# yjcaimeow/pointnerf

Hardware: AMD Instinct MI355X
Metric: Mray-samples/sec at 800x800, K=8, 2M neural points; PSNR delta vs ref (higher is better)
Workload: dtype fp32h2

## Files before the change

pointnerf_amd/csrc/aggregate_x3.hip:

```cpp
#include "agg_common.h"


namespace pnr {
namespace {

constexpr int kXT = 64;
constexpr int kXTS = kXT / kKN;
constexpr int kHidPlane = 32 * 64 * 16;
constexpr int kHidTile = 2 * kHidPlane;
constexpr int kXG = 34;
constexpr int kPG = 8;
constexpr int kPlaneX = kXG * kXT * 16;
constexpr int kPlaneP = kPG * kXT * 16;
constexpr int kP1Pitch = kHid + 4;

template <bool H>
struct XL {
  static constexpr int NPL = H ? 2 : 3;
  static constexpr int NPW = H ? 2 : 3;
  static constexpr unsigned kOne = H ? 0x3C00u : 0x3F80u;
  static constexpr int OffPE = NPL * kPlaneX;
  static constexpr int OffEx = OffPE + NPL * kPlaneP;
  static constexpr int NWB = H ? 3 : 2;
  static constexpr int OffWt = OffEx + 2 * 8 * kXT * 4;
  static constexpr int OffPr = OffWt + NWB * kXT * 4;
  static constexpr int OffSf = OffPr + 2 * kXT * 4;
  static constexpr int OffAp = OffSf + NWB * kXTS * 4;
  static constexpr int OffWa = OffAp + 4 * kXT * 4;
  static constexpr int OffH4 = OffWa + kHid * 4;
  static constexpr int OffTq = OffH4 + (H ? kXT * kP1Pitch * 4 : 0);
  static constexpr size_t Lds = (size_t)OffTq + 16;
  static_assert(OffSf % 16 == 0 && OffWa % 16 == 0 && OffH4 % 16 == 0, "16-B aligned LDS arrays");
  static_assert(kXT * kP1Pitch * 4 <= NPL * kPlaneX, "parked P1 fits the layer-input area");
  static_assert(Lds <= 160 * 1024, "LDS budget");
};

constexpr int kProducerPrio = 3;

typedef float f32x2n __attribute__((ext_vector_type(2)));
typedef float f32x4n __attribute__((ext_vector_type(4)));

struct X3Args {
  pnr_points pts;
  pnr_samples s;
  pnr_mlp w;
  SplitW wx;
  const float* p1;
  float* hid;
  int32_t* vmask;
  float* out_feat;
  float* out_weight;
  float* out_conf;
  int32_t* tile_ctr;
  pnr_agg_saved sv;
};

__device__ __forceinline__ bool xcd_mode(int64_t nt) { return nt >= 2 * (int64_t)gridDim.x + 16; }
__device__ __forceinline__ int64_t xcd_lo(int64_t nt, int x) { return nt * x / 8; }
__device__ __forceinline__ int64_t xcd_nb(int x) { return ((int)gridDim.x - x + 7) / 8; }

__device__ __forceinline__ int64_t first_tile(int64_t nt) {
  if (!xcd_mode(nt)) return blockIdx.x;
  return xcd_lo(nt, blockIdx.x & 7) + (blockIdx.x >> 3);
}

__device__ __forceinline__ int64_t take_tile(const X3Args& A, int64_t nt) {
  if (!xcd_mode(nt)) return (int64_t)gridDim.x + atomicAdd(A.tile_ctr, 1);
  const int x0 = blockIdx.x & 7;
  for (int i = 0; i < 8; ++i) {
    const int x = (x0 + i) & 7;
    const int64_t t = xcd_lo(nt, x) + xcd_nb(x) + atomicAdd(A.tile_ctr + x, 1);
    if (t < xcd_lo(nt, x + 1)) return t;
  }
  return nt;
}

__device__ __forceinline__ __amdgpu_buffer_rsrc_t rsrc(const void* base) {
  return __builtin_amdgcn_make_buffer_rsrc(const_cast<void*>(base), 0, 0x7fffffff, 0x00020000);
}

template <bool H, int NTK = 8>
__device__ __forceinline__ void load_w(uint4 (&a)[2][XL<H>::NPW], __amdgpu_buffer_rsrc_t rs, int voff, int t) {
  constexpr int NPW = XL<H>::NPW;
#pragma unroll
  for (int T = 0; T < 2; ++T)
#pragma unroll
    for (int pl = 0; pl < NPW; ++pl)
      a[T][pl] = __builtin_bit_cast(
          uint4, __builtin_amdgcn_raw_buffer_load_b128(
                     rs, voff + pl * 1024, (t * NTK + T) * NPW * 1024, 0));
}

template <bool H>
struct WRing {
  static constexpr int kWD = 3;
  uint4 a[kWD][2][XL<H>::NPW];
};

template <bool H, int NTK = 8>
__device__ __forceinline__ void prime(WRing<H>& w, __amdgpu_buffer_rsrc_t rs, int voff) {
#pragma unroll
  for (int d = 0; d < WRing<H>::kWD; ++d) load_w<H, NTK>(w.a[d], rs, voff, d);
}

template <bool H, int NTK = 8>
__device__ __forceinline__ void layer(f32x16 (&acc)[4], WRing<H>& w, __amdgpu_buffer_rsrc_t rs, int voff,
                                      const char* planes, int pstride, int nsteps, int lane) {
  constexpr int NPL = XL<H>::NPL, NPW = XL<H>::NPW, kWD = WRing<H>::kWD;
  const int c = lane & 31, h = lane >> 5;
  const char* base = planes + (h * kXT + c) * 16;
  auto ldb = [&](int t, int pt, uint4 (&bb)[NPL]) {
#pragma unroll
    for (int pl = 0; pl < NPL; ++pl)
      bb[pl] = *reinterpret_cast<const uint4*>(base + pl * pstride + (2 * t * kXT + 32 * pt) * 16);
  };
  constexpr int BD = H ? 2 : 1;
  uint4 b[BD][2][NPL];
#pragma unroll
  for (int sl = 0; sl < BD; ++sl) {
    const int t0 = sl < nsteps ? sl : nsteps - 1;
    ldb(t0, 0, b[sl][0]);
    ldb(t0, 1, b[sl][1]);
  }
  auto mm = [&](int pt, const uint4& av0, const uint4& av1, const uint4& bv) {
    if constexpr (H) {
      acc[2 * pt] = mfma_f16(av0, bv, acc[2 * pt]);
      acc[2 * pt + 1] = mfma_f16(av1, bv, acc[2 * pt + 1]);
    } else {
      acc[2 * pt] = mfma_bf16(av0, bv, acc[2 * pt]);
      acc[2 * pt + 1] = mfma_bf16(av1, bv, acc[2 * pt + 1]);
    }
  };
  auto wl = [&](uint4 (&a)[2][NPW], int pl, int tw) {
#pragma unroll
    for (int T = 0; T < 2; ++T)
      a[T][pl] = __builtin_bit_cast(
          uint4, __builtin_amdgcn_raw_buffer_load_b128(
                     rs, voff + pl * 1024, (tw * NTK + T) * NPW * 1024, 0));
  };
  auto bl = [&](int bs, int tn, int pt, int pl) {
    b[bs][pt][pl] = *reinterpret_cast<const uint4*>(base + pl * pstride + (2 * tn * kXT + 32 * pt) * 16);
  };
  uint4 scl[2];
  auto scale_next = [&](const uint4 (&an)[2][NPW], int T) {
    scl[T] = f16x8_scale2048(an[T][0]);
  };
  if constexpr (H) {
    scale_next(w.a[0], 0);
    scale_next(w.a[0], 1);
  }
  auto step_h = [&](uint4 (&a)[2][NPW], const uint4 (&an)[2][NPW], int t, int bs) {
    const int tn = t + BD < nsteps ? t + BD : nsteps - 1;
    const uint4 s0 = scl[0], s1 = scl[1];
#pragma unroll
    for (int pt = 0; pt < 2; ++pt) {
      mm(pt, s0, s1, b[bs][pt][0]);
      __builtin_amdgcn_sched_barrier(0);
      mm(pt, a[0][1], a[1][1], b[bs][pt][0]);
      __builtin_amdgcn_sched_barrier(0);
      if (pt == 1) wl(a, 1, t + kWD);
      if (pt == 0) scale_next(an, 0);
      bl(bs, tn, pt, 0);
      __builtin_amdgcn_sched_barrier(0);
      mm(pt, a[0][0], a[1][0], b[bs][pt][1]);
      __builtin_amdgcn_sched_barrier(0);
      bl(bs, tn, pt, 1);
      if (pt == 0) scale_next(an, 1);
      if (pt == 1) wl(a, 0, t + kWD);
      __builtin_amdgcn_sched_barrier(0);
    }
  };
  auto step = [&](uint4 (&a)[2][NPW], const uint4 (&an)[2][NPW], int t, int bs) {
    if constexpr (H) {
      step_h(a, an, t, bs);
    } else {
      const int tn = t + BD < nsteps ? t + BD : nsteps - 1;
#pragma unroll
      for (int pt = 0; pt < 2; ++pt) {
        mm(pt, a[0][2], a[1][2], b[bs][pt][0]);
        __builtin_amdgcn_sched_barrier(0);
        if (pt == 1) wl(a, 2, t + kWD);
        __builtin_amdgcn_sched_barrier(0);
        mm(pt, a[0][1], a[1][1], b[bs][pt][1]);
        mm(pt, a[0][0], a[1][0], b[bs][pt][2]);
        __builtin_amdgcn_sched_barrier(0);
        bl(bs, tn, pt, 2);
        __builtin_amdgcn_sched_barrier(0);
        mm(pt, a[0][1], a[1][1], b[bs][pt][0]);
        __builtin_amdgcn_sched_barrier(0);
        if (pt == 1) wl(a, 1, t + kWD);
        __builtin_amdgcn_sched_barrier(0);
        mm(pt, a[0][0], a[1][0], b[bs][pt][1]);
        __builtin_amdgcn_sched_barrier(0);
        bl(bs, tn, pt, 1);
        __builtin_amdgcn_sched_barrier(0);
        mm(pt, a[0][0], a[1][0], b[bs][pt][0]);
        __builtin_amdgcn_sched_barrier(0);
        bl(bs, tn, pt, 0);
        if (pt == 1) wl(a, 0, t + kWD);
        __builtin_amdgcn_sched_barrier(0);
      }
    }
  };
  constexpr int U = (BD == 2 && kWD % 2) ? 2 * kWD : kWD;
  int t = 0;
#pragma unroll 1
  for (; t + U <= nsteps; t += U) {
#pragma unroll
    for (int d = 0; d < U; ++d) step(w.a[d % kWD], w.a[(d + 1) % kWD], t + d, d % BD);
  }
#pragma unroll
  for (int d = 0; d < U - 1; ++d)
    if (t + d < nsteps) step(w.a[d % kWD], w.a[(d + 1) % kWD], t + d, d % BD);
}

__device__ __forceinline__ void lrelu_splith(float x0, float x1, float k, float ks, unsigned& hi, unsigned& lo) {
  typedef float f2 __attribute__((ext_vector_type(2)));
  const f2 x = {x0, x1};
  const f2 Y = __builtin_elementwise_max(x * k, x * ks);
  asm volatile(
      "v_fma_mixlo_f16 %0, %2, %4, 0\n\t"
      "v_fma_mixhi_f16 %0, %3, %4, 0\n\t"
      "v_fma_mixlo_f16 %1, %0, %5, %2 op_sel_hi:[1,0,0]\n\t"
      "v_fma_mixhi_f16 %1, %0, %5, %3 op_sel:[1,0,0] op_sel_hi:[1,0,0]"
      : "=&v"(hi), "=&v"(lo)
      : "v"(Y.x), "v"(Y.y), "s"(0x1p-11f), "s"(-2048.f));
}

template <bool H>
__device__ __forceinline__ void store_act(const f32x16 (&acc)[4], char* planes, float s, float mul, int lane,
                                          int T0, int pstride = kPlaneX) {
  const int c = lane & 31, h = lane >> 5;
  if constexpr (H) {
    const float k = 2048.f * mul, ks = k * s;
#pragma unroll
    for (int pt = 0; pt < 2; ++pt)
#pragma unroll
      for (int T = 0; T < 2; ++T)
#pragma unroll
        for (int q = 0; q < 4; ++q) {
          const f32x16& v = acc[2 * pt + T];
          unsigned a0, a1, b0, b1;
          lrelu_splith(v[4 * q], v[4 * q + 1], k, ks, a0, a1);
          lrelu_splith(v[4 * q + 2], v[4 * q + 3], k, ks, b0, b1);
          char* d = planes + ((4 * (T0 + T) + q) * kXT + 32 * pt + c) * 16 + 8 * h;
          *reinterpret_cast<uint2*>(d) = make_uint2(a0, b0);
          *reinterpret_cast<uint2*>(d + pstride) = make_uint2(a1, b1);
        }
    return;
  }
#pragma unroll
  for (int pt = 0; pt < 2; ++pt)
#pragma unroll
    for (int T = 0; T < 2; ++T)
#pragma unroll
      for (int q = 0; q < 4; ++q) {
        const f32x16& v = acc[2 * pt + T];
        unsigned a0, a1, a2, b0, b1, b2;
        split2(fmaxf(v[4 * q], s * v[4 * q]), fmaxf(v[4 * q + 1], s * v[4 * q + 1]), a0, a1, a2);
        split2(fmaxf(v[4 * q + 2], s * v[4 * q + 2]), fmaxf(v[4 * q + 3], s * v[4 * q + 3]), b0, b1, b2);
        char* d = planes + ((4 * (T0 + T) + q) * kXT + 32 * pt + c) * 16 + 8 * h;
        *reinterpret_cast<uint2*>(d) = make_uint2(a0, b0);
        *reinterpret_cast<uint2*>(d + kPlaneX) = make_uint2(a1, b1);
        *reinterpret_cast<uint2*>(d + 2 * kPlaneX) = make_uint2(a2, b2);
      }
}

template <bool H>
__device__ __forceinline__ void acc_init(f32x16 (&acc)[4], const float* bias, float inv_scale, int lane, int T0) {
  if constexpr (H) {
    const int h = lane >> 5;
#pragma unroll
    for (int T = 0; T < 2; ++T)
#pragma unroll
      for (int q = 0; q < 4; ++q) {
        const float4 b = *reinterpret_cast<const float4*>(bias + 32 * (T0 + T) + 8 * q + 4 * h);
        const float v[4] = {b.x * inv_scale, b.y * inv_scale, b.z * inv_scale, b.w * inv_scale};
#pragma unroll
        for (int i = 0; i < 4; ++i) {
          acc[T][4 * q + i] = v[i];
          acc[2 + T][4 * q + i] = v[i];
        }
      }
  } else {
#pragma unroll
    for (int i = 0; i < 4; ++i) acc[i] = (f32x16){0.f};
  }
}
constexpr int kBiasSteps(bool H) { return H ? 16 : 17; }

template <bool H>
__device__ __forceinline__ void store_group(char* planes, int pstride, int g, int pair, const float (&v)[8]) {
  if constexpr (H) {
    uint4 p0, p1;
    splith(v[0], v[1], p0.x, p1.x);
    splith(v[2], v[3], p0.y, p1.y);
    splith(v[4], v[5], p0.z, p1.z);
    splith(v[6], v[7], p0.w, p1.w);
    char* d = planes + (g * kXT + pair) * 16;
    *reinterpret_cast<uint4*>(d) = p0;
    *reinterpret_cast<uint4*>(d + pstride) = p1;
    return;
  }
  uint4 p0, p1, p2;
  split2(v[0], v[1], p0.x, p1.x, p2.x);
  split2(v[2], v[3], p0.y, p1.y, p2.y);
  split2(v[4], v[5], p0.z, p1.z, p2.z);
  split2(v[6], v[7], p0.w, p1.w, p2.w);
  char* d = planes + (g * kXT + pair) * 16;
  *reinterpret_cast<uint4*>(d) = p0;
  *reinterpret_cast<uint4*>(d + pstride) = p1;
  *reinterpret_cast<uint4*>(d + 2 * pstride) = p2;
}

struct GatherState {
  int64_t tile;
  int64_t row;
  int pid;
  float sw[3], sp[3];
  int64_t dmap;
  bool active;
};

__device__ __forceinline__ void gather_row(const X3Args& A, int64_t tile, int lane, GatherState& g) {
  const int64_t v = tile * kXTS + (lane >> 3);
  g.tile = tile;
  g.active = v < eff_n(A.s);
  g.row = g.active ? sample_row(A.s, v) : 0;
}

__device__ __forceinline__ void gather_sample(const X3Args& A, int lane, GatherState& g) {
  const int k = lane & 7, K = A.s.K;
  g.pid = (g.active && k < K) ? A.s.pidx[g.row * K + k] : -1;
#pragma unroll
  for (int a = 0; a < 3; ++a) {
    g.sw[a] = g.active ? A.s.sample_w[g.row * 3 + a] : 0.f;
    g.sp[a] = g.active ? A.s.sample_p[g.row * 3 + a] : 0.f;
  }
  g.dmap = A.s.dir_map ? (int64_t)A.s.dir_map[g.row] : g.row;
}

template <bool H, bool TR = false>
__device__ __forceinline__ void gather(const X3Args& A, const GatherState& g, int nb, int nw, char* lds, int pw, int lane,
                                       float (&dr6)[6]) {
  using L = XL<H>;
  float Rw[9];
#pragma unroll
  for (int i = 0; i < 9; ++i) Rw[i] = A.w.rw2c ? A.w.rw2c[i] : (i % 4 == 0 ? 1.f : 0.f);
// ... 130 lines not shown
    float s0, c0, s1, c1, s2, c2, s3, c3, s4, c4;
    sincosf(dr6[ch], &s0, &c0);
    sincosf(dr6[ch] * 2.f, &s1, &c1);
    sincosf(dr6[ch] * 4.f, &s2, &c2);
    sincosf(dr6[ch] * 8.f, &s3, &c3);
    sincosf(dr6[ch] * 16.f, &s4, &c4);
    pe_store<H>(lds, lane, 5 * ch + 0, s0, c0);
    pe_store<H>(lds, lane, 5 * ch + 1, s1, c1);
    pe_store<H>(lds, lane, 5 * ch + 2, s2, c2);
    pe_store<H>(lds, lane, 5 * ch + 3, s3, c3);
    pe_store<H>(lds, lane, 5 * ch + 4, s4, c4);
    if (TR && pe5) {
      const float sv[10] = {s0, c0, s1, c1, s2, c2, s3, c3, s4, c4};
#pragma unroll
      for (int i = 0; i < 10; i += 2) *reinterpret_cast<float2*>(pe5 + 10 * ch + i) = make_float2(sv[i], sv[i + 1]);
    }
  }
}

#define X3_SYNC() __syncthreads()

template <bool H, bool TR = false>
__device__ __forceinline__ void finalize_alpha(const X3Args& A, char* lds, int buf, int64_t tile, int lane) {
  using L = XL<H>;
  const int64_t n = eff_n(A.s);
  const int j = lane >> 3, k = lane & 7;
  const float* apart = reinterpret_cast<const float*>(lds + L::OffAp);
  const float* wtL = reinterpret_cast<const float*>(lds + L::OffWt) + buf * kXT;
  const int* sflag = reinterpret_cast<const int*>(lds + L::OffSf) + buf * kXTS;
  const float pa = apart[lane] + apart[kXT + lane] + apart[2 * kXT + lane] + apart[3 * kXT + lane] + A.w.ba[0];
  const float alpha_k = A.w.act_super ? softplus(pa - 1.f) : fmaxf(pa, 0.f);
  const float alpha_s = xor8_sum(wtL[lane] * alpha_k);
  const int64_t vo = tile * kXTS + j;
  if (TR && vo < n) A.sv.pa[tile * kXT + lane] = pa;
  if (k == 0 && vo < n) {
    A.vmask[vo] = sflag[j];
    if (sflag[j]) A.out_feat[vo * (kC + 1)] = alpha_s;
  }
}

template <bool H>
__device__ __forceinline__ void save_act_train(const X3Args& A, const f32x16 (&acc)[4], float* dst, int layer,
                                               int64_t tile, int64_t n, float neg, int lane, int T0, float sc) {
  const int c = lane & 31, h = lane >> 5;
#pragma unroll
  for (int pt = 0; pt < 2; ++pt) {
    const int col = 32 * pt + c;
    if (tile * kXTS + (col >> 3) >= n) continue;
    const int64_t pr = tile * kXT + col;
#pragma unroll
    for (int T = 0; T < 2; ++T) {
      f32x16 v = acc[2 * pt + T];
      if constexpr (H) v = v * sc;
      unsigned bits = 0;
#pragma unroll
      for (int q = 0; q < 4; ++q)
        *reinterpret_cast<float4*>(dst + pr * kHid + 32 * (T0 + T) + 8 * q + 4 * h) =
            make_float4(lrelu(v[4 * q], neg), lrelu(v[4 * q + 1], neg), lrelu(v[4 * q + 2], neg),
                        lrelu(v[4 * q + 3], neg));
#pragma unroll
      for (int r = 0; r < 16; ++r) bits |= (v[r] > 0.f ? 1u : 0u) << r;
      A.sv.mask[pr * 64 + 16 * layer + 2 * (T0 + T) + h] = (uint16_t)bits;
    }
  }
}

template <bool H, bool TR = false>
__device__ __forceinline__ void consumer_loop(const X3Args& A, char* lds, int wid, int lane) {
  using L = XL<H>;
  const int c = lane & 31, h = lane >> 5;
  const int64_t n = eff_n(A.s);
  const int64_t ntiles = cdiv(n, kXTS);
  const float neg = A.w.neg_slope;
  char* XP = lds;
  const char* PE = lds + L::OffPE;
  const float* P1L = reinterpret_cast<const float*>(lds);
  float* apart = reinterpret_cast<float*>(lds + L::OffAp);
  const float* waL = reinterpret_cast<const float*>(lds + L::OffWa);
  const int T0 = 2 * wid;
  const int voff = (T0 * L::NPW * 64 + lane) * 16;
  const __amdgpu_buffer_rsrc_t r1 = rsrc(A.wx.pack[0]), r2 = rsrc(A.wx.pack[1]), r3 = rsrc(A.wx.pack[2]),
                               r4 = rsrc(A.wx.pack[3]);
  const float sc1 = A.wx.scale[0], sc2 = A.wx.scale[1], sc3 = A.wx.scale[2], sc4 = A.wx.scale[3];
  WRing<H> wr;
  f32x16 acc[4];
  prime<H>(wr, r1, voff);
  X3_SYNC();
  const int* TQ = reinterpret_cast<const int*>(lds + L::OffTq);
  int it = 0;
  for (int64_t tile = first_tile(ntiles); tile < ntiles; tile = TQ[(it + 1) & 3], ++it) {
    const int buf = it & 1;
#pragma unroll
    for (int i = 0; i < 4; ++i) acc[i] = (f32x16){0.f};
    layer<H>(acc, wr, r1, voff, PE, kPlaneP, 4, lane);
    prime<H>(wr, r2, voff);
    X3_SYNC();
#pragma unroll
    for (int pt = 0; pt < 2; ++pt)
#pragma unroll
      for (int T = 0; T < 2; ++T)
#pragma unroll
        for (int q = 0; q < 4; ++q) {
          const float4 v4 = *reinterpret_cast<const float4*>(P1L + (32 * pt + c) * kP1Pitch + 32 * (T0 + T) + 8 * q +
                                                             4 * h);
          if constexpr (H) {
            acc[2 * pt + T][4 * q] = fmaf(acc[2 * pt + T][4 * q], sc1, v4.x);
            acc[2 * pt + T][4 * q + 1] = fmaf(acc[2 * pt + T][4 * q + 1], sc1, v4.y);
            acc[2 * pt + T][4 * q + 2] = fmaf(acc[2 * pt + T][4 * q + 2], sc1, v4.z);
            acc[2 * pt + T][4 * q + 3] = fmaf(acc[2 * pt + T][4 * q + 3], sc1, v4.w);
          } else {
            acc[2 * pt + T][4 * q] += v4.x;
            acc[2 * pt + T][4 * q + 1] += v4.y;
            acc[2 * pt + T][4 * q + 2] += v4.z;
            acc[2 * pt + T][4 * q + 3] += v4.w;
          }
        }
    X3_SYNC();
    store_act<H>(acc, XP, neg, 1.f, lane, T0);
    if constexpr (TR) save_act_train<H>(A, acc, A.sv.h1, 0, tile, n, neg, lane, T0, 1.f);
    if (wid == 0) {
#pragma unroll
      for (int pl = 0; pl < L::NPL; ++pl) {
        *reinterpret_cast<uint4*>(XP + pl * kPlaneX + (32 * kXT + lane) * 16) =
            make_uint4(pl == 0 ? L::kOne : 0u, 0u, 0u, 0u);
        *reinterpret_cast<uint4*>(XP + pl * kPlaneX + (33 * kXT + lane) * 16) = make_uint4(0u, 0u, 0u, 0u);
      }
    }
    acc_init<H>(acc, A.w.b2, 1.f / sc2, lane, T0);
    X3_SYNC();
    layer<H>(acc, wr, r2, voff, XP, kPlaneX, kBiasSteps(H), lane);
    prime<H>(wr, r3, voff);
    X3_SYNC();
    store_act<H>(acc, XP, neg, sc2, lane, T0);
    if constexpr (TR) save_act_train<H>(A, acc, A.sv.h2, 1, tile, n, neg, lane, T0, sc2);
    if (wid == 0) {
      const float* exL = reinterpret_cast<const float*>(lds + L::OffEx) + buf * 8 * kXT;
      float ex[8];
#pragma unroll
      for (int e = 0; e < 8; ++e) ex[e] = exL[e * kXT + lane];
      store_group<H>(XP, kPlaneX, 32, lane, ex);
    }
#pragma unroll
    for (int i = 0; i < 4; ++i) acc[i] = (f32x16){0.f};
    X3_SYNC();
    layer<H>(acc, wr, r3, voff, XP, kPlaneX, 17, lane);
    prime<H>(wr, r4, voff);
    X3_SYNC();
    store_act<H>(acc, XP, neg, sc3, lane, T0);
    if constexpr (TR) save_act_train<H>(A, acc, A.sv.h3, 2, tile, n, neg, lane, T0, sc3);
    if (wid == 0 && !H) {
#pragma unroll
      for (int pl = 0; pl < L::NPL; ++pl)
        *reinterpret_cast<uint4*>(XP + pl * kPlaneX + (32 * kXT + lane) * 16) =
            make_uint4(pl == 0 ? L::kOne : 0u, 0u, 0u, 0u);
    }
    acc_init<H>(acc, A.w.b4, 1.f / sc4, lane, T0);
    X3_SYNC();
    layer<H>(acc, wr, r4, voff, XP, kPlaneX, kBiasSteps(H), lane);
    prime<H>(wr, r1, voff);
    if constexpr (H) {
      if constexpr (TR) save_act_train<H>(A, acc, A.sv.h4, 3, tile, n, neg, lane, T0, sc4);
      float* H4 = reinterpret_cast<float*>(lds + L::OffH4);
#pragma unroll
      for (int pt = 0; pt < 2; ++pt)
#pragma unroll
        for (int T = 0; T < 2; ++T)
#pragma unroll
          for (int q = 0; q < 4; ++q) {
            const f32x16& v = acc[2 * pt + T];
            *reinterpret_cast<float4*>(H4 + (32 * pt + c) * kP1Pitch + 32 * (T0 + T) + 8 * q + 4 * h) =
                make_float4(v[4 * q], v[4 * q + 1], v[4 * q + 2], v[4 * q + 3]);
          }
    } else {
      if constexpr (TR) save_act_train<H>(A, acc, A.sv.h4, 3, tile, n, neg, lane, T0, 1.f);
      const float* wtL = reinterpret_cast<const float*>(lds + L::OffWt) + buf * kXT;
      const int* sflag = reinterpret_cast<const int*>(lds + L::OffSf) + buf * kXTS;
      float pa_part[2] = {0.f, 0.f};
      const int i8 = c & 7;
      const bool b2 = (i8 & 4) != 0, b1 = (i8 & 2) != 0, b0 = (i8 & 1) != 0;
#pragma unroll
      for (int pt = 0; pt < 2; ++pt) {
        const float wtp = wtL[32 * pt + c];
        const int sj = (32 * pt + c) >> 3;
        const int64_t vo = tile * kXTS + sj;
        const bool wrt = vo < n && sflag[sj];
#pragma unroll
        for (int T = 0; T < 2; ++T) {
          float v[16];
#pragma unroll
          for (int r = 0; r < 16; ++r) {
            const float hv = lrelu(H ? acc[2 * pt + T][r] * sc4 : acc[2 * pt + T][r], neg);
            pa_part[pt] += waL[32 * (T0 + T) + acc_row(r, h)] * hv;
            v[r] = wtp * hv;
          }
          float w8[8], w4[4], w2[2];
#pragma unroll
          for (int q = 0; q < 8; ++q) {
            const float send = b2 ? v[q] : v[q + 8];
            const float recv = __builtin_bit_cast(
                float, __builtin_amdgcn_mov_dpp(__builtin_bit_cast(int, send), 0x141, 0xf, 0xf, false));
            w8[q] = (b2 ? v[q + 8] : v[q]) + recv;
          }
#pragma unroll
          for (int q = 0; q < 4; ++q) {
            const float send = b1 ? w8[q] : w8[q + 4];
            const float recv = __builtin_bit_cast(
                float, __builtin_amdgcn_mov_dpp(__builtin_bit_cast(int, send), 0x4E, 0xf, 0xf, false));
            w4[q] = (b1 ? w8[q + 4] : w8[q]) + recv;
          }
#pragma unroll
          for (int q = 0; q < 2; ++q) {
            const float send = b0 ? w4[q] : w4[q + 2];
            const float recv = __builtin_bit_cast(
                float, __builtin_amdgcn_mov_dpp(__builtin_bit_cast(int, send), 0xB1, 0xf, 0xf, false));
            w2[q] = (b0 ? w4[q + 2] : w4[q]) + recv;
          }
          if (wrt)
            __builtin_nontemporal_store(
                (f32x2n){w2[0], w2[1]},
                reinterpret_cast<f32x2n*>(A.hid + vo * kHid + 32 * (T0 + T) + ((2 * i8) & 3) + 8 * (i8 >> 1) + 4 * h));
        }
        pa_part[pt] += __shfl_xor(pa_part[pt], 32);
      }
      if (h == 0) {
        apart[wid * kXT + c] = pa_part[0];
        apart[wid * kXT + 32 + c] = pa_part[1];
      }
    }
    X3_SYNC();
  }
}

__device__ __forceinline__ unsigned fetch_p1(f32x4n (&r)[16], const X3Args& A, const int* prow, int pw, int lane) {
  int64_t rows[16];
#pragma unroll
  for (int i = 0; i < 16; ++i) {
    const int pr = prow[16 * pw + i];
    rows[i] = pr < 0 ? -1 : (A.pts.used_map ? (int64_t)A.pts.used_map[pr] : (int64_t)pr);
  }
  unsigned empty = 0;
#pragma unroll
  for (int i = 0; i < 16; ++i) {
    r[i] = __builtin_nontemporal_load(reinterpret_cast<const f32x4n*>(A.p1 + (rows[i] < 0 ? 0 : rows[i]) * kHid) +
                                      lane);
    if (rows[i] < 0) empty |= 1u << i;
  }
  return empty;
}

__device__ __forceinline__ void park_p1(const f32x4n (&r)[16], unsigned empty, char* lds, int pw, int lane) {
  float* P1L = reinterpret_cast<float*>(lds);
#pragma unroll
  for (int i = 0; i < 16; ++i) {
    const f32x4n z = {0.f, 0.f, 0.f, 0.f};
// ... 287 lines not shown
      pe[24] = 1.f;
#pragma unroll
      for (int i = 25; i < 32; ++i) pe[i] = 0.f;
#pragma unroll
      for (int q = 0; q < 4; ++q) {
        const float g8[8] = {pe[8 * q], pe[8 * q + 1], pe[8 * q + 2], pe[8 * q + 3],
                             pe[8 * q + 4], pe[8 * q + 5], pe[8 * q + 6], pe[8 * q + 7]};
        store_group<true>(lds, kCPlane, 14 + q, lane, g8);
      }
    }
    __syncthreads();
    layer<true, 4>(acc, wr, r1b, voff, lds, kCPlane, 9, lane);
    prime<true, 4>(wr, r2, voff);
    __syncthreads();
    if (TR) save_act_rows(acc, A.hc[0], v0, n, neg, A.scale[0], lane, T0);
    store_act<true>(acc, lds, neg, A.scale[0], lane, T0, kCPlane);
    acc_init<true>(acc, A.w.bc2, 1.f / A.scale[1], lane, T0);
    __syncthreads();
    layer<true, 4>(acc, wr, r2, voff, lds, kCPlane, 8, lane);
    prime<true, 4>(wr, r3, voff);
    __syncthreads();
    if (TR) save_act_rows(acc, A.hc[1], v0, n, neg, A.scale[1], lane, T0);
    store_act<true>(acc, lds, neg, A.scale[1], lane, T0, kCPlane);
    acc_init<true>(acc, A.w.bc3, 1.f / A.scale[2], lane, T0);
    __syncthreads();
    layer<true, 4>(acc, wr, r3, voff, lds, kCPlane, 8, lane);
    prime<true, 4>(wr, r1a, voff);
    const float sc3 = A.scale[2];
    if (TR) save_act_rows(acc, A.hc[2], v0, n, neg, sc3, lane, T0);
#pragma unroll
    for (int i = 0; i < 4; ++i)
      if ((vm >> (32 * (i >> 1) + c)) & 1)
#pragma unroll
        for (int r = 0; r < 16; r += 2) chk = fmaf(0.f, acc[i][r] + acc[i][r + 1], chk);
    __syncthreads();
    float* Ob = reinterpret_cast<float*>(lds);
#pragma unroll
    for (int pt = 0; pt < 2; ++pt)
#pragma unroll
      for (int T = 0; T < 2; ++T)
#pragma unroll
        for (int q = 0; q < 4; ++q) {
          const f32x16& a = acc[2 * pt + T];
          *reinterpret_cast<float4*>(Ob + (32 * pt + c) * kOPitch + 32 * (T0 + T) + 8 * q + 4 * h) =
              make_float4(lrelu(a[4 * q] * sc3, neg), lrelu(a[4 * q + 1] * sc3, neg), lrelu(a[4 * q + 2] * sc3, neg),
                          lrelu(a[4 * q + 3] * sc3, neg));
        }
    __syncthreads();
    for (int r = wid; r < kXT; r += 2) {
      if (!((vm >> r) & 1)) continue;
      float* o = A.out_feat + (v0 + r) * (kC + 1) + 1;
      o[lane] = Ob[r * kOPitch + lane];
      o[64 + lane] = Ob[r * kOPitch + 64 + lane];
    }
    __syncthreads();
  }
  if (A.range_flag && chk != 0.f) atomicOr(A.range_flag, 1);
}

constexpr int kPG1 = 30;
constexpr int kP1Plane = kPG1 * kXT * 16;
constexpr size_t kP1H2Lds = 2 * (size_t)kP1Plane;

struct P1H2Args {
  pnr_points pts;
  const void* pack;
  float scale;
  int32_t* range_flag;
  float* p1;
  float* x1;
};

__global__ void __launch_bounds__(256) __attribute__((amdgpu_waves_per_eu(2, 2))) k_point_pre_h2(P1H2Args A) {
  extern __shared__ __attribute__((aligned(16))) char lds[];
  const int lane = threadIdx.x & 63, wid = threadIdx.x >> 6;
  const int c = lane & 31, h = lane >> 5;
  const int64_t np = p1_rows(A.pts);
  const int64_t ntiles = cdiv(np, kXT);
  const int T0 = 2 * wid;
  const int voff = (T0 * XL<true>::NPW * 64 + lane) * 16;
  const __amdgpu_buffer_rsrc_t rw = rsrc(A.pack);
  float chk = 0.f;
  WRing<true> wr;
  f32x16 acc[4];
  prime<true>(wr, rw, voff);
  for (int64_t tile = blockIdx.x; tile < ntiles; tile += gridDim.x) {
    {
      const int64_t pt = tile * kXT + lane;
      const bool act = pt < np;
      const int64_t prow = act ? (A.pts.used ? (int64_t)A.pts.used[pt] : pt) : 0;
      float e[8] = {0.f, 0.f, 0.f, 0.f, 0.f, 0.f, 0.f, 0.f};
      if (act) {
        const float4 a = reinterpret_cast<const float4*>(A.pts.emb + prow * kEmb + 8 * wid)[0];
        const float4 b = reinterpret_cast<const float4*>(A.pts.emb + prow * kEmb + 8 * wid)[1];
        e[0] = a.x; e[1] = a.y; e[2] = a.z; e[3] = a.w; e[4] = b.x; e[5] = b.y; e[6] = b.z; e[7] = b.w;
      }
      store_group<true>(lds, kP1Plane, wid, lane, e);
      if (A.x1 && act) {
        float4* xr = reinterpret_cast<float4*>(A.x1 + pt * 224 + 8 * wid);
        xr[0] = make_float4(e[0], e[1], e[2], e[3]);
        xr[1] = make_float4(e[4], e[5], e[6], e[7]);
      }
      float pe[48];
#pragma unroll
      for (int u = 0; u < 8; ++u) {
        float s0, c0;
        sincosf(e[u], &s0, &c0);
        const float s1 = 2.f * s0 * c0, c1 = (c0 - s0) * (c0 + s0);
        const float s2 = 2.f * s1 * c1, c2 = (c1 - s1) * (c1 + s1);
        pe[6 * u] = s0; pe[6 * u + 1] = c0; pe[6 * u + 2] = s1;
        pe[6 * u + 3] = c1; pe[6 * u + 4] = s2; pe[6 * u + 5] = c2;
      }
#pragma unroll
      for (int g = 0; g < 6; ++g) {
        const float g8[8] = {pe[8 * g], pe[8 * g + 1], pe[8 * g + 2], pe[8 * g + 3],
                             pe[8 * g + 4], pe[8 * g + 5], pe[8 * g + 6], pe[8 * g + 7]};
        store_group<true>(lds, kP1Plane, 4 + 6 * wid + g, lane, g8);
      }
      if (A.x1 && act) {
        float4* xr = reinterpret_cast<float4*>(A.x1 + pt * 224 + 32 + 48 * wid);
#pragma unroll
        for (int q = 0; q < 12; ++q) xr[q] = make_float4(pe[4 * q], pe[4 * q + 1], pe[4 * q + 2], pe[4 * q + 3]);
      }
      if (wid == 0) {
        const float one[8] = {1.f, 0.f, 0.f, 0.f, 0.f, 0.f, 0.f, 0.f};
        const float zero[8] = {0.f, 0.f, 0.f, 0.f, 0.f, 0.f, 0.f, 0.f};
        store_group<true>(lds, kP1Plane, 28, lane, one);
        store_group<true>(lds, kP1Plane, 29, lane, zero);
      }
    }
    __syncthreads();
#pragma unroll
    for (int i = 0; i < 4; ++i) acc[i] = (f32x16){0.f};
    layer<true>(acc, wr, rw, voff, lds, kP1Plane, 15, lane);
    prime<true>(wr, rw, voff);
#pragma unroll
    for (int pt = 0; pt < 2; ++pt) {
      const int64_t prow = tile * kXT + 32 * pt + c;
#pragma unroll
      for (int T = 0; T < 2; ++T)
#pragma unroll
        for (int q = 0; q < 4; ++q) {
          const f32x16& v = acc[2 * pt + T];
          const float4 o = make_float4(v[4 * q] * A.scale, v[4 * q + 1] * A.scale, v[4 * q + 2] * A.scale,
                                       v[4 * q + 3] * A.scale);
          chk = fmaf(0.f, (o.x + o.y) + (o.z + o.w), chk);
          if (prow < np)
            *reinterpret_cast<float4*>(A.p1 + prow * kHid + 32 * (T0 + T) + 8 * q + 4 * h) = o;
        }
    }
    __syncthreads();
  }
  if (A.range_flag && chk != 0.f) atomicOr(A.range_flag, 1);
}

}

int launch_point_pre_h2(const pnr_points& pts, const void* pack, float scale, int32_t* range_flag, float* p1,
                        hipStream_t st, float* x1) {
  static bool attr = false;
  if (!attr) {
    PNR_HIP(hipFuncSetAttribute(reinterpret_cast<const void*>(&k_point_pre_h2),
                                hipFuncAttributeMaxDynamicSharedMemorySize, (int)kP1H2Lds));
    attr = true;
  }
  P1H2Args a;
  a.pts = pts;
  a.pack = pack;
  a.scale = scale;
  a.range_flag = range_flag;
  a.p1 = p1;
  a.x1 = x1;
  const int64_t np = pts.used ? pts.n_used : pts.n;
  hipLaunchKernelGGL(k_point_pre_h2, dim3(grid_for(cdiv(np, kXT), 1, 256 * 2)), dim3(256), kP1H2Lds, st, a);
  PNR_LAUNCH_CHECK();
  return PNR_OK;
}

int launch_color_h2(const pnr_samples& s, const pnr_mlp& w, const void* const pack[4], const float scale[3],
                    int32_t* range_flag, const float* hid, const int32_t* vmask, float* out_feat, hipStream_t st,
                    const float* rw2c_pp, const pnr_agg_saved* train) {
  static bool attr = false;
  if (!attr) {
    PNR_HIP(hipFuncSetAttribute(reinterpret_cast<const void*>(&k_color_h2<false>),
                                hipFuncAttributeMaxDynamicSharedMemorySize, (int)kColH2Lds));
    PNR_HIP(hipFuncSetAttribute(reinterpret_cast<const void*>(&k_color_h2<true>),
                                hipFuncAttributeMaxDynamicSharedMemorySize, (int)kColH2Lds));
    attr = true;
  }
  ColH2Args a;
  a.s = s;
  a.w = w;
  for (int i = 0; i < 4; ++i) a.pack[i] = pack[i];
  for (int i = 0; i < 3; ++i) a.scale[i] = scale[i];
  a.range_flag = range_flag;
  a.hid = hid;
  a.vmask = vmask;
  a.out_feat = out_feat;
  a.rw2c_pp = rw2c_pp;
  a.hid_rows = train ? train->hid : nullptr;
  a.vpe = train ? train->vpe : nullptr;
  a.hc[0] = train ? train->hc1 : nullptr;
  a.hc[1] = train ? train->hc2 : nullptr;
  a.hc[2] = train ? train->hc3 : nullptr;
  const dim3 grid(grid_for(cdiv(s.n_max, kXT), 1, 256 * 4));
  if (train) hipLaunchKernelGGL(k_color_h2<true>, grid, dim3(128), kColH2Lds, st, a);
  else hipLaunchKernelGGL(k_color_h2<false>, grid, dim3(128), kColH2Lds, st, a);
  PNR_LAUNCH_CHECK();
  return PNR_OK;
}


template <bool H>
int launch_pairs_split(const pnr_points& pts, const pnr_samples& s, const pnr_mlp& w, const SplitW& wx,
                       const float* p1, float* hid, int32_t* vmask, float* out_feat, float* out_weight,
                       float* out_conf, int32_t* tile_ctr, hipStream_t st, const pnr_agg_saved* sv) {
  const void* fn = H ? (sv ? reinterpret_cast<const void*>(&k_pairs_h2_train) : reinterpret_cast<const void*>(&k_pairs_h2))
                     : (sv ? reinterpret_cast<const void*>(&k_pairs_x3_train) : reinterpret_cast<const void*>(&k_pairs_x3));
  static bool attr[2] = {false, false};
  if (!attr[sv ? 1 : 0]) {
    PNR_HIP(hipFuncSetAttribute(fn, hipFuncAttributeMaxDynamicSharedMemorySize, (int)XL<H>::Lds));
    attr[sv ? 1 : 0] = true;
  }
  X3Args a;
  a.pts = pts;
  a.s = s;
  a.w = w;
  a.wx = wx;
// ... 31 lines not shown
```

Baseline: 819.1.

## Use separate main and correction accumulators for f16 split MFMA layers

For the f16 two-plane weight split, the hi-plane product goes into its own accumulator set and the lo-plane products into a second correction set. The two sets are folded with a single fma (main*2048 + corr) at store time. This replaces the per-step rescaling of weights by 2048 (the scale_next VALU work) and starts from zero accumulators instead of explicit zeroing. The cost is 64 more accumulator VGPRs per lane, which risks spills or lower occupancy under the fixed waves-per-EU bound, and it changes how rounding errors accumulate.

```diff
diff --git a/pointnerf_amd/csrc/aggregate_x3.hip b/pointnerf_amd/csrc/aggregate_x3.hip
--- a/pointnerf_amd/csrc/aggregate_x3.hip
+++ b/pointnerf_amd/csrc/aggregate_x3.hip
@@ -103,9 +103,11 @@
   for (int d = 0; d < WRing<H>::kWD; ++d) load_w<H, NTK>(w.a[d], rs, voff, d);
 }
 
-template <bool H, int NTK = 8>
-__device__ __forceinline__ void layer(f32x16 (&acc)[4], WRing<H>& w, __amdgpu_buffer_rsrc_t rs, int voff,
-                                      const char* planes, int pstride, int nsteps, int lane) {
+template <bool H, int NTK = 8, bool ACC2 = false, bool ZACC = false>
+__device__ __forceinline__ void layer(f32x16 (&acc)[4], f32x16 (&corr)[4], WRing<H>& w, __amdgpu_buffer_rsrc_t rs,
+                                      int voff, const char* planes, int pstride, int nsteps, int lane) {
+  static_assert(ACC2 || !ZACC, "zero-start accumulators: with two accumulator sets only");
+  static_assert(H || !ACC2, "two accumulator sets: the f16 split only");
   constexpr int NPL = XL<H>::NPL, NPW = XL<H>::NPW, kWD = WRing<H>::kWD;
   const int c = lane & 31, h = lane >> 5;
   const char* base = planes + (h * kXT + c) * 16;
@@ -122,8 +124,13 @@
     ldb(t0, 0, b[sl][0]);
     ldb(t0, 1, b[sl][1]);
   }
-  auto mm = [&](int pt, const uint4& av0, const uint4& av1, const uint4& bv) {
-    if constexpr (H) {
+  auto mm = [&](int pt, const uint4& av0, const uint4& av1, const uint4& bv, bool to_corr = false, bool zc = false) {
+    if constexpr (ACC2) {
+      f32x16 (&d)[4] = to_corr ? corr : acc;
+      const f32x16 z = {0.f};
+      d[2 * pt] = mfma_f16(av0, bv, zc ? z : d[2 * pt]);
+      d[2 * pt + 1] = mfma_f16(av1, bv, zc ? z : d[2 * pt + 1]);
+    } else if constexpr (H) {
       acc[2 * pt] = mfma_f16(av0, bv, acc[2 * pt]);
       acc[2 * pt + 1] = mfma_f16(av1, bv, acc[2 * pt + 1]);
     } else {
@@ -143,26 +150,26 @@
   };
   uint4 scl[2];
   auto scale_next = [&](const uint4 (&an)[2][NPW], int T) {
-    scl[T] = f16x8_scale2048(an[T][0]);
+    if constexpr (!ACC2) scl[T] = f16x8_scale2048(an[T][0]);
   };
   if constexpr (H) {
     scale_next(w.a[0], 0);
     scale_next(w.a[0], 1);
   }
-  auto step_h = [&](uint4 (&a)[2][NPW], const uint4 (&an)[2][NPW], int t, int bs) {
+  auto step_h = [&](uint4 (&a)[2][NPW], const uint4 (&an)[2][NPW], int t, int bs, bool first = false) {
     const int tn = t + BD < nsteps ? t + BD : nsteps - 1;
-    const uint4 s0 = scl[0], s1 = scl[1];
+    const uint4 s0 = ACC2 ? a[0][0] : scl[0], s1 = ACC2 ? a[1][0] : scl[1];
 #pragma unroll
     for (int pt = 0; pt < 2; ++pt) {
-      mm(pt, s0, s1, b[bs][pt][0]);
+      mm(pt, s0, s1, b[bs][pt][0], false, first && ZACC);
       __builtin_amdgcn_sched_barrier(0);
-      mm(pt, a[0][1], a[1][1], b[bs][pt][0]);
+      mm(pt, a[0][1], a[1][1], b[bs][pt][0], true, first);
       __builtin_amdgcn_sched_barrier(0);
       if (pt == 1) wl(a, 1, t + kWD);
       if (pt == 0) scale_next(an, 0);
       bl(bs, tn, pt, 0);
       __builtin_amdgcn_sched_barrier(0);
-      mm(pt, a[0][0], a[1][0], b[bs][pt][1]);
+      mm(pt, a[0][0], a[1][0], b[bs][pt][1], true);
       __builtin_amdgcn_sched_barrier(0);
       bl(bs, tn, pt, 1);
       if (pt == 0) scale_next(an, 1);
@@ -203,16 +210,26 @@
     }
   };
   constexpr int U = (BD == 2 && kWD % 2) ? 2 * kWD : kWD;
-  int t = 0;
+  constexpr int P = ACC2 ? 1 : 0;
+  if constexpr (ACC2) step_h(w.a[0], w.a[1 % kWD], 0, 0, true);
+  int t = P;
 #pragma unroll 1
   for (; t + U <= nsteps; t += U) {
 #pragma unroll
-    for (int d = 0; d < U; ++d) step(w.a[d % kWD], w.a[(d + 1) % kWD], t + d, d % BD);
+    for (int d = 0; d < U; ++d) step(w.a[(d + P) % kWD], w.a[(d + P + 1) % kWD], t + d, (d + P) % BD);
   }
 #pragma unroll
   for (int d = 0; d < U - 1; ++d)
-    if (t + d < nsteps) step(w.a[d % kWD], w.a[(d + 1) % kWD], t + d, d % BD);
-}
+    if (t + d < nsteps) step(w.a[(d + P) % kWD], w.a[(d + P + 1) % kWD], t + d, (d + P) % BD);
+}
+
+template <bool H, int NTK = 8>
+__device__ __forceinline__ void layer(f32x16 (&acc)[4], WRing<H>& w, __amdgpu_buffer_rsrc_t rs, int voff,
+                                      const char* planes, int pstride, int nsteps, int lane) {
+  layer<H, NTK, false>(acc, acc, w, rs, voff, planes, pstride, nsteps, lane);
+}
+
+__device__ __forceinline__ float fold2(float main, float corr) { return fmaf(main, 2048.f, corr); }
 
 __device__ __forceinline__ void lrelu_splith(float x0, float x1, float k, float ks, unsigned& hi, unsigned& lo) {
   typedef float f2 __attribute__((ext_vector_type(2)));
@@ -227,9 +244,9 @@
       : "v"(Y.x), "v"(Y.y), "s"(0x1p-11f), "s"(-2048.f));
 }
 
-template <bool H>
-__device__ __forceinline__ void store_act(const f32x16 (&acc)[4], char* planes, float s, float mul, int lane,
-                                          int T0, int pstride = kPlaneX) {
+template <bool H, bool ACC2 = false>
+__device__ __forceinline__ void store_act(const f32x16 (&acc)[4], const f32x16 (&corr)[4], char* planes, float s,
+                                          float mul, int lane, int T0, int pstride = kPlaneX) {
   const int c = lane & 31, h = lane >> 5;
   if constexpr (H) {
     const float k = 2048.f * mul, ks = k * s;
@@ -239,10 +256,13 @@
       for (int T = 0; T < 2; ++T)
 #pragma unroll
         for (int q = 0; q < 4; ++q) {
-          const f32x16& v = acc[2 * pt + T];
+          float v[4];
+#pragma unroll
+          for (int i = 0; i < 4; ++i)
+            v[i] = ACC2 ? fold2(acc[2 * pt + T][4 * q + i], corr[2 * pt + T][4 * q + i]) : acc[2 * pt + T][4 * q + i];
           unsigned a0, a1, b0, b1;
-          lrelu_splith(v[4 * q], v[4 * q + 1], k, ks, a0, a1);
-          lrelu_splith(v[4 * q + 2], v[4 * q + 3], k, ks, b0, b1);
+          lrelu_splith(v[0], v[1], k, ks, a0, a1);
+          lrelu_splith(v[2], v[3], k, ks, b0, b1);
           char* d = planes + ((4 * (T0 + T) + q) * kXT + 32 * pt + c) * 16 + 8 * h;
           *reinterpret_cast<uint2*>(d) = make_uint2(a0, b0);
           *reinterpret_cast<uint2*>(d + pstride) = make_uint2(a1, b1);
@@ -264,6 +284,12 @@
         *reinterpret_cast<uint2*>(d + kPlaneX) = make_uint2(a1, b1);
         *reinterpret_cast<uint2*>(d + 2 * kPlaneX) = make_uint2(a2, b2);
       }
+}
+
+template <bool H>
+__device__ __forceinline__ void store_act(const f32x16 (&acc)[4], char* planes, float s, float mul, int lane,
+                                          int T0, int pstride = kPlaneX) {
+  store_act<H, false>(acc, acc, planes, s, mul, lane, T0, pstride);
 }
 
 template <bool H>
@@ -560,17 +586,25 @@
   const __amdgpu_buffer_rsrc_t r1 = rsrc(A.wx.pack[0]), r2 = rsrc(A.wx.pack[1]), r3 = rsrc(A.wx.pack[2]),
                                r4 = rsrc(A.wx.pack[3]);
   const float sc1 = A.wx.scale[0], sc2 = A.wx.scale[1], sc3 = A.wx.scale[2], sc4 = A.wx.scale[3];
+  constexpr bool A2 = H && !TR;
+  const float in2 = A2 ? 0x1p-11f : 1.f;
   WRing<H> wr;
   f32x16 acc[4];
+  f32x16 corr[4];
+  auto zero_acc = [&]() {
+    if constexpr (!A2) {
+#pragma unroll
+      for (int i = 0; i < 4; ++i) acc[i] = (f32x16){0.f};
+    }
+  };
   prime<H>(wr, r1, voff);
   X3_SYNC();
   const int* TQ = reinterpret_cast<const int*>(lds + L::OffTq);
   int it = 0;
   for (int64_t tile = first_tile(ntiles); tile < ntiles; tile = TQ[(it + 1) & 3], ++it) {
     const int buf = it & 1;
-#pragma unroll
-    for (int i = 0; i < 4; ++i) acc[i] = (f32x16){0.f};
-    layer<H>(acc, wr, r1, voff, PE, kPlaneP, 4, lane);
+    zero_acc();
+    layer<H, 8, A2, A2>(acc, corr, wr, r1, voff, PE, kPlaneP, 4, lane);
     prime<H>(wr, r2, voff);
     X3_SYNC();
 #pragma unroll
@@ -581,7 +615,13 @@
         for (int q = 0; q < 4; ++q) {
           const float4 v4 = *reinterpret_cast<const float4*>(P1L + (32 * pt + c) * kP1Pitch + 32 * (T0 + T) + 8 * q +
                                                              4 * h);
-          if constexpr (H) {
+          if constexpr (A2) {
+            const float v[4] = {v4.x, v4.y, v4.z, v4.w};
+#pragma unroll
+            for (int i = 0; i < 4; ++i)
+              acc[2 * pt + T][4 * q + i] =
+                  fmaf(acc[2 * pt + T][4 * q + i], 2048.f * sc1, fmaf(corr[2 * pt + T][4 * q + i], sc1, v[i]));
+          } else if constexpr (H) {
             acc[2 * pt + T][4 * q] = fmaf(acc[2 * pt + T][4 * q], sc1, v4.x);
             acc[2 * pt + T][4 * q + 1] = fmaf(acc[2 * pt + T][4 * q + 1], sc1, v4.y);
             acc[2 * pt + T][4 * q + 2] = fmaf(acc[2 * pt + T][4 * q + 2], sc1, v4.z);
@@ -604,12 +644,12 @@
         *reinterpret_cast<uint4*>(XP + pl * kPlaneX + (33 * kXT + lane) * 16) = make_uint4(0u, 0u, 0u, 0u);
       }
     }
-    acc_init<H>(acc, A.w.b2, 1.f / sc2, lane, T0);
-    X3_SYNC();
-    layer<H>(acc, wr, r2, voff, XP, kPlaneX, kBiasSteps(H), lane);
+    acc_init<H>(acc, A.w.b2, in2 / sc2, lane, T0);
+    X3_SYNC();
+    layer<H, 8, A2>(acc, corr, wr, r2, voff, XP, kPlaneX, kBiasSteps(H), lane);
     prime<H>(wr, r3, voff);
     X3_SYNC();
-    store_act<H>(acc, XP, neg, sc2, lane, T0);
+    store_act<H, A2>(acc, corr, XP, neg, sc2, lane, T0);
     if constexpr (TR) save_act_train<H>(A, acc, A.sv.h2, 1, tile, n, neg, lane, T0, sc2);
     if (wid == 0) {
       const float* exL = reinterpret_cast<const float*>(lds + L::OffEx) + buf * 8 * kXT;
@@ -618,13 +658,12 @@
       for (int e = 0; e < 8; ++e) ex[e] = exL[e * kXT + lane];
       store_group<H>(XP, kPlaneX, 32, lane, ex);
     }
-#pragma unroll
-    for (int i = 0; i < 4; ++i) acc[i] = (f32x16){0.f};
-    X3_SYNC();
-    layer<H>(acc, wr, r3, voff, XP, kPlaneX, 17, lane);
+    zero_acc();
+    X3_SYNC();
+    layer<H, 8, A2, A2>(acc, corr, wr, r3, voff, XP, kPlaneX, 17, lane);
     prime<H>(wr, r4, voff);
     X3_SYNC();
-    store_act<H>(acc, XP, neg, sc3, lane, T0);
+    store_act<H, A2>(acc, corr, XP, neg, sc3, lane, T0);
     if constexpr (TR) save_act_train<H>(A, acc, A.sv.h3, 2, tile, n, neg, lane, T0, sc3);
     if (wid == 0 && !H) {
 #pragma unroll
@@ -632,9 +671,9 @@
         *reinterpret_cast<uint4*>(XP + pl * kPlaneX + (32 * kXT + lane) * 16) =
             make_uint4(pl == 0 ? L::kOne : 0u, 0u, 0u, 0u);
     }
-    acc_init<H>(acc, A.w.b4, 1.f / sc4, lane, T0);
-    X3_SYNC();
-    layer<H>(acc, wr, r4, voff, XP, kPlaneX, kBiasSteps(H), lane);
+    acc_init<H>(acc, A.w.b4, in2 / sc4, lane, T0);
+    X3_SYNC();
+    layer<H, 8, A2>(acc, corr, wr, r4, voff, XP, kPlaneX, kBiasSteps(H), lane);
     prime<H>(wr, r1, voff);
     if constexpr (H) {
       if constexpr (TR) save_act_train<H>(A, acc, A.sv.h4, 3, tile, n, neg, lane, T0, sc4);
@@ -645,9 +684,12 @@
         for (int T = 0; T < 2; ++T)
 #pragma unroll
           for (int q = 0; q < 4; ++q) {
-            const f32x16& v = acc[2 * pt + T];
+            float v[4];
+#pragma unroll
+            for (int i = 0; i < 4; ++i)
+              v[i] = A2 ? fold2(acc[2 * pt + T][4 * q + i], corr[2 * pt + T][4 * q + i]) : acc[2 * pt + T][4 * q + i];
             *reinterpret_cast<float4*>(H4 + (32 * pt + c) * kP1Pitch + 32 * (T0 + T) + 8 * q + 4 * h) =
-                make_float4(v[4 * q], v[4 * q + 1], v[4 * q + 2], v[4 * q + 3]);
+                make_float4(v[0], v[1], v[2], v[3]);
           }
     } else {
       if constexpr (TR) save_act_train<H>(A, acc, A.sv.h4, 3, tile, n, neg, lane, T0, 1.f);
@@ -1101,7 +1143,7 @@
   const __amdgpu_buffer_rsrc_t rw = rsrc(A.pack);
   float chk = 0.f;
   WRing<true> wr;
-  f32x16 acc[4];
+  f32x16 acc[4], corr[4];
   prime<true>(wr, rw, voff);
   for (int64_t tile = blockIdx.x; tile < ntiles; tile += gridDim.x) {
     {
@@ -1149,9 +1191,7 @@
       }
     }
     __syncthreads();
-#pragma unroll
-    for (int i = 0; i < 4; ++i) acc[i] = (f32x16){0.f};
-    layer<true>(acc, wr, rw, voff, lds, kP1Plane, 15, lane);
+    layer<true, 8, true, true>(acc, corr, wr, rw, voff, lds, kP1Plane, 15, lane);
     prime<true>(wr, rw, voff);
 #pragma unroll
     for (int pt = 0; pt < 2; ++pt) {
@@ -1160,9 +1200,11 @@
       for (int T = 0; T < 2; ++T)
 #pragma unroll
         for (int q = 0; q < 4; ++q) {
-          const f32x16& v = acc[2 * pt + T];
-          const float4 o = make_float4(v[4 * q] * A.scale, v[4 * q + 1] * A.scale, v[4 * q + 2] * A.scale,
-                                       v[4 * q + 3] * A.scale);
+          const f32x16& m = acc[2 * pt + T];
+          const f32x16& r = corr[2 * pt + T];
+          const float4 o = make_float4(fold2(m[4 * q], r[4 * q]) * A.scale, fold2(m[4 * q + 1], r[4 * q + 1]) * A.scale,
+                                       fold2(m[4 * q + 2], r[4 * q + 2]) * A.scale,
+                                       fold2(m[4 * q + 3], r[4 * q + 3]) * A.scale);
           chk = fmaf(0.f, (o.x + o.y) + (o.z + o.w), chk);
           if (prow < np)
             *reinterpret_cast<float4*>(A.p1 + prow * kHid + 32 * (T0 + T) + 8 * q + 4 * h) = o;
```

Result: faster. 829.7 (median of 6 runs) (+1.3%).
